# jepsen-io/maelstrom

Hardware: AMD Instinct MI355X
Metric: simulated_msgs_per_sec (histories/sec passing checker in histories_per_sec) (higher is better)
Workload: dtype u32

## Files before the change

maelstrom_amd/csrc/checker.hip:

```cpp
#include <hip/hip_runtime.h>

#include <cstring>
#include <vector>

#include "engine_internal.h"

#define NONE 0xFFFFu
#define NONE32 0xFFFFFFFFu
#define NOLAT 0xFFFFFFFFu

struct CParams {
  const msim_op *rows;
  const u32 *payload;
  const msim_inst_meta *meta;
  msim_check_result *out;
  u32 *recs;
  u32 max_rows, max_pay, max_values, C, workload, max_reads;
  u32 off_valid, off_tbl;
  float rcp_C;
};

#ifdef MSIM_HIPEMU
struct __attribute__((packed, aligned(4))) ck_u32x4 { u32 x, y, z, w; };
#else
// ... 339 lines not shown
      while (lo < hi) {
        const u32 mid = lo + (hi - lo) / 2;
        u32 c = 0;
        for (u32 e = lane; e < v_cur; e += 64) { const u32 l = lat[e]; c += (l != NOLAT && l <= mid) ? 1u : 0u; }
        if (c_wave_sum(c) > want) hi = mid; else lo = mid + 1;
      }
      q[qi] = lo;
    }
  }

  if (lane == 0) {
    msim_check_result o;
    o.attempt_count = v_cur; o.stable_count = n_stable; o.lost_count = n_lost; o.never_read_count = n_never;
    o.stale_count = n_stale; o.duplicated_count = 0; o.error_count = errors;
    for (int i = 0; i < 5; i++) o.stable_latency_ms[i] = q[i];
#ifdef CK_PROF
    o.stable_latency_ms[0] = (u32)(ck_t1 - ck_t0); o.stable_latency_ms[1] = (u32)(ck_t2 - ck_t1); o.stable_latency_ms[2] = (u32)(__builtin_readcyclecounter() - ck_t2); o.stable_latency_ms[3] = ck_rounds; o.stable_latency_ms[4] = n_ri;
#endif
    o.op_count = op_count; o.ok_count = n_ok; o.fail_count = n_fail; o.info_count = n_info;
    if (meta.flags) o.valid = 0;
    else if (!setfull) o.valid = errors == 0 ? 1 : 0;
    else o.valid = n_lost ? 0u : (n_stable == 0 ? 2u : 1u);
    p.out[inst] = o;
  }
}

static size_t check_lds_layout(CParams &cp) {
  size_t lds = (size_t)cp.max_values * 3 * 2 < (size_t)cp.max_values * 4 ? (size_t)cp.max_values * 4 : (size_t)cp.max_values * 3 * 2;
  lds = (lds + 3) & ~(size_t)3;
  cp.off_valid = (u32)lds;
  lds += ((size_t)(cp.max_reads + 31) / 32 + 2) * 4;
  cp.off_tbl = (u32)lds;
  lds += (size_t)cp.C * 3 * 4;
  return lds;
}

static const char *check_limits(u32 max_rows, u32 max_values, u32 concurrency) {
  if (max_rows >= 0xFFFF || max_values > 2048 || concurrency > 128 || concurrency == 0) return "device checker: max_rows must be < 65535, max_values <= 2048, concurrency 1..128";
  return nullptr;
}

static hipError_t check_dispatch(CParams &cp, u32 n, hipStream_t st) {
  cp.max_reads = cp.max_rows / 2 + 1;
  cp.rcp_C = 1.0f / (float)cp.C;
  const size_t lds = check_lds_layout(cp);
  if (lds > 64 * 1024) {
    const hipError_t e = hipFuncSetAttribute(reinterpret_cast<const void *>(&check_kernel), hipFuncAttributeMaxDynamicSharedMemorySize, (int)lds);
    if (e != hipSuccess) return e;
  }
  hipLaunchKernelGGL(check_kernel, dim3(n), dim3(64), lds, st, cp);
  return hipGetLastError();
}

int msim_check_launch(msim_ctx *ctx) {
  MSIM_HIP_TRY(ctx, hipSetDevice(ctx->device));
  const msim_config &c = ctx->cfg;
  CParams cp;
  std::memset(&cp, 0, sizeof cp);
  cp.rows = ctx->d_rows; cp.payload = ctx->d_payload; cp.meta = ctx->d_meta; cp.out = ctx->d_check;
  cp.max_rows = c.max_rows; cp.max_pay = c.max_payload_words; cp.max_values = c.max_values; cp.C = c.concurrency; cp.workload = c.workload;
  if (const char *why = check_limits(c.max_rows, c.max_values, c.concurrency)) { ctx->err = why; return MSIM_E_UNSUPPORTED; }
  const size_t rec_bytes = (size_t)ctx->n_inst * (c.max_rows / 2 + 1) * 3 * sizeof(u32);
  if (ctx->cap_check_scratch < rec_bytes) {
    if (ctx->d_check_scratch) (void)msim_dev_free(ctx->d_check_scratch);
    ctx->d_check_scratch = nullptr; ctx->cap_check_scratch = 0;
    MSIM_HIP_TRY(ctx, msim_dev_malloc(&ctx->d_check_scratch, rec_bytes));
    ctx->cap_check_scratch = rec_bytes;
  }
  cp.recs = static_cast<u32 *>(ctx->d_check_scratch);
  MSIM_HIP_TRY(ctx, hipEventRecord(ctx->ev2, ctx->stream));
  MSIM_HIP_TRY(ctx, check_dispatch(cp, ctx->n_inst, ctx->stream));
  MSIM_HIP_TRY(ctx, hipEventRecord(ctx->ev3, ctx->stream));
  MSIM_HIP_TRY(ctx, hipEventSynchronize(ctx->ev3));
  MSIM_HIP_TRY(ctx, hipEventElapsedTime(&ctx->check_ms, ctx->ev2, ctx->ev3));
  ctx->checked = true; ctx->check_fetched = false;
  return MSIM_OK;
}

extern "C" int msim_check_set_full_batch(int device, uint32_t workload, uint32_t concurrency, const msim_op *rows, const uint32_t *n_rows, uint32_t max_rows,
                                         const uint32_t *payload, uint32_t max_payload_words, uint32_t max_values, uint32_t n_histories, msim_check_result *out) {
  if (!rows || !n_rows || !out || n_histories == 0 || max_rows == 0 || (!payload && max_payload_words)) return MSIM_E_INVALID;
  if (workload != MSIM_WL_ECHO && workload != MSIM_WL_BROADCAST && workload != MSIM_WL_G_SET) return MSIM_E_INVALID;
  if (check_limits(max_rows, max_values, concurrency)) return MSIM_E_UNSUPPORTED;
  if (hipSetDevice(device) != hipSuccess) return MSIM_E_HIP;
  std::vector<msim_inst_meta> hm(n_histories);
  for (u32 i = 0; i < n_histories; i++) { std::memset(&hm[i], 0, sizeof hm[i]); if (n_rows[i] > max_rows) return MSIM_E_RANGE; hm[i].n_rows = n_rows[i]; }
  CParams cp;
  std::memset(&cp, 0, sizeof cp);
  cp.max_rows = max_rows; cp.max_pay = max_payload_words; cp.max_values = max_values; cp.C = concurrency; cp.workload = workload;
  msim_op *d_rows = nullptr; u32 *d_pay = nullptr; msim_inst_meta *d_meta = nullptr; msim_check_result *d_out = nullptr; u32 *d_rec = nullptr;
  const size_t pay_bytes = (size_t)n_histories * (max_payload_words ? max_payload_words : 1) * sizeof(u32);
  int rc = MSIM_E_HIP;
  do {
    if (msim_dev_malloc(&d_rows, (size_t)n_histories * max_rows * sizeof(msim_op)) != hipSuccess) break;
    if (msim_dev_malloc(&d_pay, pay_bytes) != hipSuccess) break;
    if (msim_dev_malloc(&d_meta, (size_t)n_histories * sizeof(msim_inst_meta)) != hipSuccess) break;
    if (msim_dev_malloc(&d_out, (size_t)n_histories * sizeof(msim_check_result)) != hipSuccess) break;
    if (msim_dev_malloc(&d_rec, (size_t)n_histories * (max_rows / 2 + 1) * 3 * sizeof(u32)) != hipSuccess) break;
    if (hipMemcpy(d_rows, rows, (size_t)n_histories * max_rows * sizeof(msim_op), hipMemcpyHostToDevice) != hipSuccess) break;
    if (max_payload_words && hipMemcpy(d_pay, payload, pay_bytes, hipMemcpyHostToDevice) != hipSuccess) break;
    if (hipMemcpy(d_meta, hm.data(), (size_t)n_histories * sizeof(msim_inst_meta), hipMemcpyHostToDevice) != hipSuccess) break;
    cp.rows = d_rows; cp.payload = d_pay; cp.meta = d_meta; cp.out = d_out; cp.recs = d_rec;
    if (check_dispatch(cp, n_histories, nullptr) != hipSuccess) break;
    if (hipDeviceSynchronize() != hipSuccess) break;
    if (hipMemcpy(out, d_out, (size_t)n_histories * sizeof(msim_check_result), hipMemcpyDeviceToHost) != hipSuccess) break;
    rc = MSIM_OK;
  } while (false);
  for (void *q : {(void *)d_rows, (void *)d_pay, (void *)d_meta, (void *)d_out, (void *)d_rec}) if (q) (void)msim_dev_free(q);
  return rc;
}

__global__ void __launch_bounds__(64) availability_kernel(const msim_op *rows, const msim_inst_meta *meta, u32 max_rows, uint2 *out) {
  const u32 lane = threadIdx.x, inst = blockIdx.x;
  const u32 n = meta[inst].n_rows;
  const uint4 *r = reinterpret_cast<const uint4 *>(rows + (size_t)inst * max_rows);
  u32 ok = 0, inv = 0;
  for (u32 i = lane; i < n; i += 64) { const u32 t = r[i].z & 3u; ok += t == MSIM_T_OK; inv += t == MSIM_T_INVOKE; }
  ok = c_wave_sum(ok); inv = c_wave_sum(inv);
  if (lane == 0) out[inst] = make_uint2(ok, inv);
}

static void availability_verdict(uint32_t ok, uint32_t inv, uint32_t mode, double a, msim_availability *o) {
  o->ok_count = ok; o->invoke_count = inv;
  o->ok_fraction = inv == 0 ? 1.0f : (float)((double)ok / (double)inv);
  o->valid = mode == MSIM_AVAIL_NIL ? 1u : mode == MSIM_AVAIL_TOTAL ? (o->ok_fraction == 1.0f ? 1u : 0u) : (a <= (double)o->ok_fraction ? 1u : 0u);
}

extern "C" int msim_check_availability_rows(const msim_op *rows, uint32_t n_rows, uint32_t mode, double availability, msim_availability *out) {
  if ((!rows && n_rows) || !out || mode > MSIM_AVAIL_FRACTION || (mode == MSIM_AVAIL_FRACTION && !(availability >= 0.0 && availability <= 1.0))) return MSIM_E_INVALID;
// ... 27 lines not shown
```

maelstrom_amd/csrc/engine.hip:

```cpp
#include <hip/hip_runtime.h>
#include <cstdlib>

#include <cstdio>
#include <cstring>
#include <new>
#include <vector>


#include "sim_kernels.h"

__device__ u32 wave_min_ref(u32 v) { for (int o = 32; o; o >>= 1) v = min(v, (u32)__shfl_xor((int)v, o)); return v; }
__device__ u32 wave_incl_scan_ref(u32 v) {
  const u32 lane = threadIdx.x & 63;
  for (int o = 1; o < 64; o <<= 1) { u32 t = (u32)__shfl_up((int)v, o); if (lane >= (u32)o) v += t; }
  return v;
}
__global__ void wave_selftest_kernel(const u32 *in, u32 *out) {
  const u32 lane = threadIdx.x;
  const u32 v = in[blockIdx.x * 64 + lane];
  u32 bad = 0;
  bad |= wave_min(v) != wave_min_ref(v);
  bad |= wave_incl_scan(v & 0xFFFF) != wave_incl_scan_ref(v & 0xFFFF);
  bad |= wave_sum(v & 0xFF) != rdlane(wave_incl_scan_ref(v & 0xFF), 63);
  bad |= (lane < 32) && scan32(v & 0xFFFF) != wave_incl_scan_ref(v & 0xFFFF);
// ... 37 lines not shown
  if (c->d_gpay) (void)msim_dev_free(c->d_gpay);
  if (c->d_goff) (void)msim_dev_free(c->d_goff);
  c->d_grows = c->d_gpay = nullptr; c->d_goff = nullptr; c->cap_grows = c->cap_gpay = c->cap_goff = 0;
  c->d_compact = nullptr; c->d_off = nullptr;
  c->cap_compact = c->cap_off = c->cap_h_rows = c->cap_h_payload = c->cap_h_journal = c->cap_h_meta = 0;
  delete[] c->h_row_off; delete[] c->h_pay_off; delete[] c->h_ev_off;
  c->d_journal = nullptr; c->h_journal = nullptr; c->h_ev_off = nullptr;
  c->d_rows = nullptr; c->d_payload = nullptr; c->d_stats = nullptr; c->d_meta = nullptr; c->d_scratch = nullptr; c->d_check = nullptr;
  c->h_rows = nullptr; c->h_payload = nullptr; c->h_stats = nullptr; c->h_meta = nullptr; c->h_check = nullptr;
  c->h_row_off = nullptr; c->h_pay_off = nullptr;
  c->cap_inst = 0;
}

extern "C" int msim_create(const msim_config *cfg, int device, msim_ctx **out, char *err, size_t errlen) {
  if (!cfg || !out) { set_err(err, errlen, "null argument"); return MSIM_E_INVALID; }
  *out = nullptr;
  msim_config c = *cfg;
  int rc = msim_config_finalize(&c, err, errlen);
  if (rc != MSIM_OK) return rc;
  const bool dt_many = (c.node_program == MSIM_NODE_TXN_DATOMIC || c.node_program == MSIM_NODE_TXN_MULTI_KEY) && c.concurrency > c.n_nodes;
  if ((c.node_program == MSIM_NODE_TXN_MULTI_KEY || c.node_program == MSIM_NODE_TXN_DATOMIC) && !dt_many && (c.concurrency != c.n_nodes || c.n_nodes > 30)) {
    set_err(err, errlen, "multi_key_txn / datomic: one worker per node and at most 30 nodes (two service lanes), or k x node-count workers with nodes + workers + 2 <= 64");
    return MSIM_E_UNSUPPORTED;
  }
  if (dt_many && c.n_nodes + c.concurrency + 2 > 64) { set_err(err, errlen, "multi_key_txn / datomic with several workers per node: nodes + workers + 2 services <= 64"); return MSIM_E_UNSUPPORTED; }
  const bool txn_many = (c.node_program == MSIM_NODE_TXN_SINGLE_KEY || c.node_program == MSIM_NODE_KAFKA) && c.concurrency > c.n_nodes;
  if (c.node_program == MSIM_NODE_BCAST_BATCH && (c.n_nodes > 32 || c.n_nodes + (c.concurrency > c.n_nodes ? c.concurrency : c.n_nodes) > 64)) {
    set_err(err, errlen, "broadcast-batch: one cluster per wavefront only: n_nodes <= 32 and n_nodes + max(concurrency, n_nodes) <= 64");
    return MSIM_E_UNSUPPORTED;
  }
  const uint32_t slots = (c.concurrency > c.n_nodes ? c.concurrency : c.n_nodes) + (dt_many ? 2 : txn_many ? 1 : 0);
  const bool wide_prog = c.node_program == MSIM_NODE_G_SET || c.node_program == MSIM_NODE_BCAST_FF || c.node_program == MSIM_NODE_BCAST_FF_ECHOBACK ||
                         c.node_program == MSIM_NODE_BCAST_ACK_RETRY || c.node_program == MSIM_NODE_BCAST_RPC_ALL || c.node_program == MSIM_NODE_PN_COUNTER;
  const bool wide = c.n_nodes > 32 && c.n_nodes <= 127 && wide_prog && c.concurrency == c.n_nodes;
  const uint32_t svc_lanes = c.node_program == MSIM_NODE_LIN_KV_PROXY || c.node_program == MSIM_NODE_TSO_IDS ? 1 : 0;
  if (!wide && (c.n_nodes > 32 || c.n_nodes + slots + svc_lanes > 64)) {
    set_err(err, errlen, "this build maps one cluster to one wavefront: n_nodes <= 32 and n_nodes + max(concurrency, n_nodes) <= 64 "
                         "(g-set, the counters and the broadcast programs with concurrency == n_nodes: up to 127 nodes)");
    return MSIM_E_UNSUPPORTED;
  }
  int ndev = 0;
  if (hipGetDeviceCount(&ndev) != hipSuccess || ndev <= 0) {
    set_err(err, errlen, "no HIP device visible: libmaelsim has no CPU path"); return MSIM_E_NO_DEVICE; }
  if (device < 0 || device >= ndev) { set_err(err, errlen, "device index out of range"); return MSIM_E_INVALID; }
  msim_ctx *ctx = new (std::nothrow) msim_ctx();
  if (!ctx) return MSIM_E_NOMEM;
  ctx->cfg = c; ctx->device = device;
  hipError_t e = hipSetDevice(device);
  if (e == hipSuccess) e = hipStreamCreateWithFlags(&ctx->stream, hipStreamNonBlocking);
  if (e == hipSuccess) e = hipEventCreate(&ctx->ev0);
  if (e == hipSuccess) e = hipEventCreate(&ctx->ev1);
  if (e == hipSuccess) e = hipEventCreate(&ctx->ev2);
  if (e == hipSuccess) e = hipEventCreate(&ctx->ev3);
  if (e != hipSuccess) { set_err(err, errlen, hipGetErrorString(e)); delete ctx; return MSIM_E_HIP; }
  *out = ctx;
  return MSIM_OK;
}

static uint32_t mk_tcap(const msim_config &c) {
  const double ops = (double)c.rate_mhz * (double)c.time_limit_ms / 1e6 * 1.125 + 64.0;
  uint32_t t = 64; while (t < 4.0 * ops * c.max_txn_length / c.n_nodes + 64.0) t <<= 1;
  return t;
}
static uint32_t mk_ccap(const msim_config &c) { return 4 * mk_tcap(c); }

static uint32_t raft_log_cap(const msim_config &c) {
  const double expected = (double)c.rate_mhz * (double)c.time_limit_ms / 1e6;
  return (uint32_t)(expected + expected / 8.0) + 64 + 8;
}
static uint64_t proto_scratch_words(const msim_config &c) {
  uint64_t w = 4;
  if (c.node_program == MSIM_NODE_RAFT) w = (uint64_t)c.n_nodes * raft_log_cap(c) * 2 + (uint64_t)c.n_nodes * R_ARENA_WORDS;
  if (c.node_program == MSIM_NODE_BCAST_ACK_RETRY) w = (uint64_t)c.n_nodes * c.max_values * 3;
  if (c.node_program == MSIM_NODE_BCAST_BATCH) w = (uint64_t)c.n_nodes * (c.max_values / 2) + (uint64_t)c.n_nodes * c.n_nodes * 4;
  if (c.node_program == MSIM_NODE_TXN_SINGLE_KEY) w = (uint64_t)c.max_values * (c.max_writes_per_key + 1);
  if (c.node_program == MSIM_NODE_TXN_MULTI_KEY)
    w = (uint64_t)c.max_values * (c.max_writes_per_key + 4 + 2 * (c.max_writes_per_key + 1)) + (uint64_t)c.n_nodes * mk_ccap(c) + (uint64_t)c.n_nodes * mk_tcap(c) / 4 + 4 +
        (uint64_t)c.n_nodes * ((c.concurrency > c.n_nodes ? MKG_SLOTS : MK_SLOTS) - MK_SL) * mk_slot_words(8);
  if (c.node_program == MSIM_NODE_TXN_DATOMIC) w = dt_scratch_words(c);
  if (c.node_program == MSIM_NODE_KAFKA) w = (uint64_t)KF_KEYS * (2 * (c.max_writes_per_key + 1) + 1);
  if (c.node_program == MSIM_NODE_TXN_RW_HAT) {
    const uint64_t G = c.max_rows / 2;
    w = (uint64_t)c.n_nodes * c.max_values + 2 * G + ((uint64_t)c.n_nodes * G + 3) / 4 + c.replication_words;
  }
  if (c.node_program == MSIM_NODE_G_SET || c.node_program == MSIM_NODE_PN_COUNTER) {
    const uint64_t total_ms = (uint64_t)c.time_limit_ms + c.quiesce_ms + 2ull * c.client_timeout_ms;
    const uint64_t ticks = total_ms / 5000 + 3;
    w = ticks * c.n_nodes * (c.max_values / 32);
    if (c.n_nodes > 32) w = ((w + ticks * (c.max_values / 32) + 3) & ~3ull) + (c.node_program == MSIM_NODE_G_SET ? wide_sparse_words(ticks, c.max_values / 32) : 0) + (((uint64_t)c.n_nodes * (c.max_values / 32) + 3) & ~3ull);
  }
  const bool bcast_ff = c.node_program == MSIM_NODE_BCAST_FF || c.node_program == MSIM_NODE_BCAST_FF_ECHOBACK;
  const bool bcast_rpc = c.node_program == MSIM_NODE_BCAST_ACK_RETRY || c.node_program == MSIM_NODE_BCAST_RPC_ALL;
  if (bcast_ff && c.n_nodes > 32) w = 4 + (((uint64_t)c.n_nodes * (c.max_values / 32) + 3) & ~3ull);
  if (bcast_rpc && c.n_nodes > 32) w = (uint64_t)c.n_nodes * c.max_values * 6 + (((uint64_t)c.n_nodes * (c.max_values / 32) + 3) & ~3ull);
  return (w + 3) & ~3ull;
}
static uint64_t scratch_words(const msim_config &c) {
  const uint64_t queues = c.n_nodes + (c.node_program == MSIM_NODE_KAFKA || c.node_program == MSIM_NODE_TXN_SINGLE_KEY || c.node_program == MSIM_NODE_LIN_KV_PROXY || c.node_program == MSIM_NODE_TSO_IDS ? 1 : c.node_program == MSIM_NODE_TXN_MULTI_KEY || c.node_program == MSIM_NODE_TXN_DATOMIC ? 2 : 0);
  uint64_t w = proto_scratch_words(c) + queues * c.spill_capacity * 4;
  if (c.node_program == MSIM_NODE_LIN_KV_PROXY || c.node_program == MSIM_NODE_TSO_IDS) w += (uint64_t)(c.concurrency > c.n_nodes ? c.concurrency : c.n_nodes) * (R_CLIENT_CAP - PX_CL) * 4;
  if (msim_raft4_eligible(c)) w += msim_raft4_extra_scratch_words(c);
  if (msim_svc4_eligible(c)) w += msim_svc4_extra_scratch_words(c);
  if (msim_txng4_eligible(c)) w += msim_txng4_extra_scratch_words(c);
  if (msim_dtg4_eligible(c)) w += msim_dtg4_extra_scratch_words(c);
  if (msim_txn8_eligible(c)) w += msim_txn8_extra_scratch_words(c);
  if (msim_mk8_eligible(c)) w += msim_mk8_extra_scratch_words(c);
  if (msim_dt8_eligible(c)) w += msim_dt8_extra_scratch_words(c);
  if (msim_hat8_eligible(c)) w += msim_hat8_extra_scratch_words(c);
  if (msim_kafka8_eligible(c)) w += msim_kafka8_extra_scratch_words(c);
  if (msim_uid8_eligible(c)) w += msim_uid8_extra_scratch_words(c);
  if (msim_crdt8_eligible(c)) w += msim_crdt8_extra_scratch_words(c);
  if (msim_bcast8_eligible(c)) w += msim_bcast8_extra_scratch_words(c);
  if (msim_duo_eligible(c)) w = ((w + 31) & ~31ull) + msim_duo_extra_scratch_words(c);
  return w;
}

static int ensure_buffers(msim_ctx *ctx, uint32_t n) {
  if (n <= ctx->cap_inst) return MSIM_OK;
  free_buffers(ctx);
  const msim_config &c = ctx->cfg;
  ctx->scratch_words_per_inst = scratch_words(c);
  MSIM_HIP_TRY(ctx, msim_dev_malloc(&ctx->d_rows, (size_t)n * c.max_rows * sizeof(msim_op)));
  MSIM_HIP_TRY(ctx, msim_dev_malloc(&ctx->d_payload, (size_t)n * c.max_payload_words * 4));
  MSIM_HIP_TRY(ctx, msim_dev_malloc(&ctx->d_stats, (size_t)n * sizeof(msim_net_stats)));
  MSIM_HIP_TRY(ctx, msim_dev_malloc(&ctx->d_meta, (size_t)n * sizeof(msim_inst_meta)));
  MSIM_HIP_TRY(ctx, msim_dev_malloc(&ctx->d_scratch, (size_t)n * ctx->scratch_words_per_inst * 4));
  MSIM_HIP_TRY(ctx, msim_dev_malloc(&ctx->d_check, (size_t)n * sizeof(msim_check_result)));
  if (c.journal_capacity) MSIM_HIP_TRY(ctx, msim_dev_malloc(&ctx->d_journal, (size_t)n * c.journal_capacity * sizeof(msim_event)));
  ctx->cap_inst = n;
  return MSIM_OK;
}

static int run_impl(msim_ctx *ctx, uint64_t first, uint32_t n, hipStream_t st, bool blocking) {
  if (!ctx) return MSIM_E_INVALID;
  if (n == 0) { ctx->err = "n_instances must be > 0"; return MSIM_E_INVALID; }
  MSIM_HIP_TRY(ctx, hipSetDevice(ctx->device));
  if (ctx->fetch_pending) { MSIM_HIP_TRY(ctx, hipStreamSynchronize(ctx->stream)); ctx->fetch_pending = false; }
  int rc = ensure_buffers(ctx, n);
  if (rc != MSIM_OK) return rc;
  const msim_config &c = ctx->cfg;
  KParams kp;
  std::memset(&kp, 0, sizeof kp);
  kp.cfg = c; kp.first_instance = first;
  kp.rows = ctx->d_rows; kp.payload = ctx->d_payload; kp.stats = ctx->d_stats; kp.meta = ctx->d_meta;
  kp.scratch = ctx->d_scratch; kp.scratch_words = ctx->scratch_words_per_inst;
  kp.journal = reinterpret_cast<uint4 *>(ctx->d_journal);
  kp.N = c.n_nodes; kp.C = c.concurrency; kp.CS = c.concurrency > c.n_nodes ? c.concurrency : c.n_nodes;
  kp.W = c.max_values / 32;
  kp.cap_node = c.inbox_capacity; kp.spill_cap = c.spill_capacity; kp.spill_off = proto_scratch_words(c);
  const uint64_t period_us = 1000000000ull / (c.rate_mhz ? c.rate_mhz : 1);
  if (2 * period_us > 0xFFFFFFFFull || 2000ull * c.nemesis_interval_ms > 0xFFFFFFFFull) { ctx->err = "rate too low / nemesis interval too long for u32 microseconds"; return MSIM_E_INVALID; }
  kp.gen_period2_us = (u32)(2 * period_us);
  kp.nem_period2_us = (u32)(2000ull * c.nemesis_interval_ms);
  const bool is_raft = c.node_program == MSIM_NODE_RAFT;
  kp.raft_log_cap = is_raft ? raft_log_cap(c) : 0;
  kp.dev_flags = msim_dev_flags(ctx);
  const bool wide = c.n_nodes > 32;
  const bool wide_setl = wide_sets_in_lds(c, kp.dev_flags);
  const bool wide_crdt = wide && (c.node_program == MSIM_NODE_G_SET || c.node_program == MSIM_NODE_PN_COUNTER);
  size_t off = (wide_setl || wide_crdt) ? 0 : (wide ? WIDE_STAGE_ROWS : STAGE_ROWS) * 16;
  const bool is_txn = c.node_program == MSIM_NODE_TXN_SINGLE_KEY, is_px = c.node_program == MSIM_NODE_LIN_KV_PROXY || c.node_program == MSIM_NODE_TSO_IDS;
  const bool is_hat = c.node_program == MSIM_NODE_TXN_RW_HAT, is_mk = c.node_program == MSIM_NODE_TXN_MULTI_KEY, is_kf = c.node_program == MSIM_NODE_KAFKA, is_dt = c.node_program == MSIM_NODE_TXN_DATOMIC;
  kp.mk_tcap = is_mk ? mk_tcap(c) : is_dt ? dt_tcap(c) : 0; kp.mk_ccap = is_mk ? mk_ccap(c) : 0;
  kp.off_inbox = (u32)off;
  const bool dt_many = (is_dt || is_mk) && c.concurrency > c.n_nodes;
  const bool txn_many = (is_txn || is_kf) && c.concurrency > c.n_nodes;
  off += (is_mk || is_dt) ? ((size_t)(kp.N + 2) * kp.cap_node + (size_t)(dt_many ? kp.CS : kp.N) * T_CLIENT_CAP) * 16 : is_hat ? ((size_t)kp.N * kp.cap_node + (size_t)kp.CS * T_CLIENT_CAP) * 16    : is_px ? ((size_t)(kp.N + 1) * kp.cap_node + (size_t)kp.CS * PX_CL) * 16 : (is_txn || is_kf) ? ((size_t)(kp.N + 1) * kp.cap_node + (size_t)(txn_many ? kp.CS : kp.N) * T_CLIENT_CAP) * 16
                : ((size_t)kp.N * kp.cap_node + (size_t)kp.CS * (is_raft ? R_CLIENT_CAP : CLIENT_INBOX_CAP)) * 16 + wide_client_bytes(c);
  kp.off_seen = (u32)off;
  off += is_mk ? ((size_t)kp.N * MK_SL * mk_slot_words(mk_keys_for(c)) + (size_t)kp.N * mk_keys_for(c) * 3 + 36) * 4
       : is_dt ? ((size_t)kp.N * (dt_many ? DG_WORDS : DC_WORDS) + 36) * 4
       : is_hat ? 36 * 4
       : is_px ? (size_t)kp.N * PX_SLOTS * 8 + ((c.node_program == MSIM_NODE_LIN_KV_PROXY && c.proxy_service == MSIM_SVC_SEQ_KV) ? 34 : 2) * 256 + 64 * 4
       : is_txn ? (size_t)kp.N * (txn_many ? TG_SLOTS : TXN_SLOTS) * 16 + 36 * 4
       : is_kf ? ((size_t)kp.N * (txn_many ? KFG_SLOTS : KF_SLOTS) * KSW + (size_t)kp.N * KF_KEYS + (size_t)(txn_many ? kp.CS : kp.N) * KF_KEYS + 36 + 2 * KF_KEYS) * 4
       : is_raft ? (size_t)kp.N * 256 + (size_t)kp.N * kp.N * 3 * 4
       : wide ? (wide_setl ? (size_t)kp.N * kp.W * 4 : 0) + wide_pending_bytes(c)
                 : (size_t)kp.N * kp.W * 4;
  off = (off + 15) & ~(size_t)15;
  kp.off_misc = (u32)off; if (c.nemesis_mask) off += (wide ? 128 : 64) * 4;
  const size_t lds = off;
  if (lds > 160 * 1024) { ctx->err = "cluster state exceeds the 160 KiB LDS of a CU (lower inbox_capacity / max_values)"; return MSIM_E_INVALID; }

  static const int poison = []() { const char *p = std::getenv("MSIM_POISON"); return p ? (int)(std::strtoul(p, nullptr, 0) & 0xFFu) : -1; }();
  if (poison >= 0) {
    MSIM_HIP_TRY(ctx, hipMemsetAsync(ctx->d_rows, poison, (size_t)ctx->cap_inst * c.max_rows * sizeof(msim_op), st));
    MSIM_HIP_TRY(ctx, hipMemsetAsync(ctx->d_payload, poison, (size_t)ctx->cap_inst * c.max_payload_words * 4, st));
    MSIM_HIP_TRY(ctx, hipMemsetAsync(ctx->d_stats, poison, (size_t)ctx->cap_inst * sizeof(msim_net_stats), st));
    MSIM_HIP_TRY(ctx, hipMemsetAsync(ctx->d_meta, poison, (size_t)ctx->cap_inst * sizeof(msim_inst_meta), st));
    MSIM_HIP_TRY(ctx, hipMemsetAsync(ctx->d_scratch, poison, (size_t)ctx->cap_inst * ctx->scratch_words_per_inst * 4, st));
    MSIM_HIP_TRY(ctx, hipMemsetAsync(ctx->d_check, poison, (size_t)ctx->cap_inst * sizeof(msim_check_result), st));
    if (ctx->d_journal) MSIM_HIP_TRY(ctx, hipMemsetAsync(ctx->d_journal, poison, (size_t)ctx->cap_inst * c.journal_capacity * sizeof(msim_event), st));
    if (ctx->d_check_scratch) MSIM_HIP_TRY(ctx, hipMemsetAsync(ctx->d_check_scratch, poison, ctx->cap_check_scratch, st));
    if (ctx->d_perf_scratch) MSIM_HIP_TRY(ctx, hipMemsetAsync(ctx->d_perf_scratch, poison, ctx->cap_perf_scratch, st));
  }
  MSIM_HIP_TRY(ctx, hipEventRecord(ctx->ev0, st));
  hipError_t e;
  const char *kname = "?";
  auto took = [&](hipError_t r, const char *k) { if (r != MSIM_LAYOUT_DOES_NOT_FIT) kname = k; return r; };
  e = MSIM_LAYOUT_DOES_NOT_FIT;
  if (msim_duo_eligible(c) && !(kp.dev_flags & 0x200u) && !((kp.dev_flags & 0x8000u) && msim_bcast8_eligible(c))) {
    e = took(msim_launch_duo(kp, n, st), "duo");
    if (e == MSIM_LAYOUT_DOES_NOT_FIT && (kp.dev_flags & 0x400u)) { ctx->err = "MSIM_DEV_FLAGS bit 10: the two-clusters-per-wavefront layout was required but this cluster state does not fit it"; return MSIM_E_UNSUPPORTED; }
  }
  if (e == MSIM_LAYOUT_DOES_NOT_FIT && msim_bcast8_eligible(c) && !(kp.dev_flags & 0x200u)) e = took(msim_launch_bcast8(kp, n, st), "bcast8");
  if (msim_raft4_eligible(c) && !(kp.dev_flags & 0x200u)) e = took(msim_launch_raft4(kp, n, st), "raft4");
  if (msim_svc4_eligible(c) && !(kp.dev_flags & 0x200u)) e = took(msim_launch_svc4(kp, n, st), c.node_program == MSIM_NODE_TSO_IDS ? "svc4<TSO>" : "svc4");
  if (msim_txng4_eligible(c) && !(kp.dev_flags & 0x200u)) e = took(msim_launch_txng4(kp, n, st), "txng4");
  if (msim_dtg4_eligible(c) && !(kp.dev_flags & 0x200u)) e = took(msim_launch_dtg4(kp, n, st), "dtg4");
  if (msim_txn8_eligible(c) && !(kp.dev_flags & 0x200u)) e = took(msim_launch_txn8(kp, n, st), "txn8");
  if (msim_mk8_eligible(c) && !(kp.dev_flags & 0x200u)) e = took(msim_launch_mk8(kp, n, st), "mk8");
  if (msim_dt8_eligible(c) && !(kp.dev_flags & 0x200u)) e = took(msim_launch_dt8(kp, n, st), "dt8");
  if (msim_hat8_eligible(c) && !(kp.dev_flags & 0x200u)) e = took(msim_launch_hat8(kp, n, st), "hat8");
  if (msim_kafka8_eligible(c) && !(kp.dev_flags & 0x200u)) e = took(msim_launch_kafka8(kp, n, st), "kafka8");
  if (msim_uid8_eligible(c) && !(kp.dev_flags & 0x200u)) e = took(msim_launch_uid8(kp, n, st), "uid8");
  if (msim_crdt8_eligible(c) && !(kp.dev_flags & 0x200u)) e = took(msim_launch_crdt8(kp, n, st), "crdt8");
  if (e == MSIM_LAYOUT_DOES_NOT_FIT && (kp.dev_flags & 0x400u) && is_raft) { ctx->err = "MSIM_DEV_FLAGS bit 10: the four-clusters-per-wavefront Raft layout was required but does not apply"; return MSIM_E_UNSUPPORTED; }
  if (e == MSIM_LAYOUT_DOES_NOT_FIT) switch (c.node_program) {
    case MSIM_NODE_ECHO: case MSIM_NODE_FLAKE_IDS: e = took(msim_launch_general_a(kp, n, lds, st), "general_a"); break;
    case MSIM_NODE_G_SET: e = wide ? took(msim_launch_wide_gset(kp, n, lds, st), "wide_gset") : took(msim_launch_general_a(kp, n, lds, st), "general_a"); break;
    case MSIM_NODE_PN_COUNTER: e = wide ? took(msim_launch_wide_pn(kp, n, lds, st), "wide_pn") : took(msim_launch_general_a(kp, n, lds, st), "general_a"); break;
    case MSIM_NODE_BCAST_FF: case MSIM_NODE_BCAST_FF_ECHOBACK: e = wide ? took(msim_launch_wide_bcast(kp, n, lds, st), "wide_bcast") : took(msim_launch_general_b(kp, n, lds, st), "general_b"); break;
    case MSIM_NODE_BCAST_ACK_RETRY: case MSIM_NODE_BCAST_RPC_ALL: e = wide ? took(msim_launch_wide_ack(kp, n, lds, st), "wide_ack") : took(msim_launch_general_c(kp, n, lds, st), "general_c"); break;
    case MSIM_NODE_BCAST_BATCH: e = took(msim_launch_general_d(kp, n, lds, st), "general_d"); break;
    case MSIM_NODE_RAFT: e = took(msim_launch_raft1(kp, n, lds, st), "raft1"); break;
    case MSIM_NODE_LIN_KV_PROXY: case MSIM_NODE_TSO_IDS: e = took(msim_launch_svc1(kp, n, lds, st), "svc1"); break;
    case MSIM_NODE_TXN_SINGLE_KEY: e = txn_many ? took(msim_launch_txng(kp, n, lds, st), "txng") : took(msim_launch_txn1(kp, n, lds, st), "txn1"); break;
    case MSIM_NODE_TXN_MULTI_KEY: e = dt_many ? took(msim_launch_mkg(kp, n, lds, st), "mkg") : took(msim_launch_mk1(kp, n, lds, st), "mk1"); break;
    case MSIM_NODE_TXN_DATOMIC: e = dt_many ? took(msim_launch_dtg(kp, n, lds, st), "dtg") : took(msim_launch_dt1(kp, n, lds, st), "dt1"); break;
    case MSIM_NODE_KAFKA: e = txn_many ? took(msim_launch_kafkag(kp, n, lds, st), "kafkag") : took(msim_launch_kafka1(kp, n, lds, st), "kafka1"); break;
    case MSIM_NODE_TXN_RW_HAT: e = c.concurrency > c.n_nodes ? took(msim_launch_hatg(kp, n, lds, st), "hatg") : took(msim_launch_hat1(kp, n, lds, st), "hat1"); break;
    default: ctx->err = "node program not built into this engine"; return MSIM_E_UNSUPPORTED;
  }
  if (kp.dev_flags & 0x1000u) std::fprintf(stderr, "[layout] %s %u\n", kname, n);
  if (e != hipSuccess) { ctx->err = std::string("kernel launch: ") + hipGetErrorString(e); return MSIM_E_HIP; }
  ctx->n_inst = n; ctx->first_instance = first;
  ctx->fetched = false; ctx->fetch_pending = false; ctx->checked = false; ctx->check_fetched = false; ctx->ran = true;
  MSIM_HIP_TRY(ctx, hipEventRecord(ctx->ev1, st));
  ctx->sim_ms_stale = true;
  if (blocking) {
    MSIM_HIP_TRY(ctx, hipEventSynchronize(ctx->ev1));
    MSIM_HIP_TRY(ctx, hipEventElapsedTime(&ctx->sim_ms, ctx->ev0, ctx->ev1));
    ctx->sim_ms_stale = false;
  }
  return MSIM_OK;
}

extern "C" int msim_run(msim_ctx *ctx, uint64_t first_instance, uint32_t n_instances) {
  if (!ctx) return MSIM_E_INVALID;
  return run_impl(ctx, first_instance, n_instances, ctx->stream, true);
}

extern "C" int msim_run_async(msim_ctx *ctx, uint64_t first_instance, uint32_t n_instances, void *hip_stream) {
  if (!ctx) return MSIM_E_INVALID;
  return run_impl(ctx, first_instance, n_instances, hip_stream ? (hipStream_t)hip_stream : ctx->stream, false);
}

extern "C" int msim_check(msim_ctx *ctx) {
  if (!ctx) return MSIM_E_INVALID;
  if (!ctx->ran) { ctx->err = "msim_check before msim_run"; return MSIM_E_RANGE; }
  if (ctx->cfg.workload == MSIM_WL_LIN_KV) {
    return (msim_dev_flags(ctx) & 0x800u) ?
           msim_check_lin_kv_host(ctx) : msim_check_lin_kv_device(ctx);
  }
  if (ctx->cfg.workload == MSIM_WL_TXN_LIST_APPEND) {
    return (msim_dev_flags(ctx) & 0x800u) ?
           msim_check_txn_host(ctx) : msim_check_txn_device(ctx);
  }
  if (ctx->cfg.workload == MSIM_WL_TXN_RW_REGISTER) {
    return (msim_dev_flags(ctx) & 0x800u) ?
           msim_check_txn_host(ctx) : msim_check_rw_device(ctx);
  }
  if (ctx->cfg.workload == MSIM_WL_KAFKA) {
    return (msim_dev_flags(ctx) & 0x800u) ?
           msim_check_kafka_host(ctx) : msim_check_kafka_device(ctx);
  }
  if (ctx->cfg.workload == MSIM_WL_PN_COUNTER || ctx->cfg.workload == MSIM_WL_G_COUNTER) {
    return (msim_dev_flags(ctx) & 0x800u) ?
           msim_check_pn_host(ctx) : msim_check_pn_device(ctx);
  }
  if (ctx->cfg.workload == MSIM_WL_UNIQUE_IDS) {
    return (msim_dev_flags(ctx) & 0x800u) ?
           msim_check_unique_host(ctx) : msim_check_unique_device(ctx);
  }
  return msim_check_launch(ctx);
}

__global__ void __launch_bounds__(256) compact_kernel(const uint4 *__restrict__ src, uint4 *__restrict__ dst, const uint64_t *__restrict__ off,
                                                      uint64_t stride_units) {
  const u32 i = blockIdx.x;
  const uint64_t o = off[i], cnt = off[i + 1] - o;
  const uint4 *s = src + (size_t)i * stride_units;
  for (uint64_t k = (uint64_t)blockIdx.y * 256 + threadIdx.x; k < cnt; k += (uint64_t)gridDim.y * 256) dst[o + k] = s[k];
}
__global__ void __launch_bounds__(256) compact_words_kernel(const u32 *__restrict__ src, u32 *__restrict__ dst, const uint64_t *__restrict__ off,
                                                            uint64_t stride_words) {
  const u32 i = blockIdx.x;
  const uint64_t o = off[i], cnt = off[i + 1] - o;
  const u32 *s = src + (size_t)i * stride_words;
  for (uint64_t k = (uint64_t)blockIdx.y * 256 + threadIdx.x; k < cnt; k += (uint64_t)gridDim.y * 256) dst[o + k] = s[k];
}

template <typename T>
static int grow_pinned(msim_ctx *ctx, T **buf, size_t *cap, size_t bytes) {
  if (*buf && *cap >= bytes) return MSIM_OK;
  if (*buf) { (void)hipHostFree(*buf); *buf = nullptr; *cap = 0; }
  const size_t want = bytes + bytes / 8 + 4096;
  MSIM_HIP_TRY(ctx, hipHostMalloc(reinterpret_cast<void **>(buf), want));
  *cap = want;
  return MSIM_OK;
}

static int fetch_compacted(msim_ctx *ctx, const void *d_src, uint64_t stride_units, bool units16, const uint64_t *h_off, void *h_dst, int pair, int phase) {
  const uint32_t n = ctx->n_inst;
  const uint64_t total = h_off[n];
  if (!total) return MSIM_OK;
  void **d_compact = pair ? &ctx->d_compact2 : &ctx->d_compact; size_t *cap_compact = pair ? &ctx->cap_compact2 : &ctx->cap_compact;
  uint64_t **d_off = pair ? &ctx->d_off2 : &ctx->d_off; size_t *cap_off = pair ? &ctx->cap_off2 : &ctx->cap_off;
  const size_t unit = units16 ? 16 : 4, bytes = (size_t)total * unit;
  if (phase == 1) { MSIM_HIP_TRY(ctx, hipMemcpyAsync(h_dst, *d_compact, bytes, hipMemcpyDeviceToHost, ctx->stream)); return MSIM_OK; }
  if (*cap_compact < bytes) {
    if (*d_compact) (void)msim_dev_free(*d_compact);
    *d_compact = nullptr; *cap_compact = 0;
    MSIM_HIP_TRY(ctx, msim_dev_malloc(d_compact, bytes + bytes / 8));
    *cap_compact = bytes + bytes / 8;
  }
  if (*cap_off < (size_t)(n + 1) * 8) {
    if (*d_off) (void)msim_dev_free(*d_off);
    *d_off = nullptr; *cap_off = 0;
    MSIM_HIP_TRY(ctx, msim_dev_malloc(reinterpret_cast<void **>(d_off), (size_t)(n + 1) * 8));
    *cap_off = (size_t)(n + 1) * 8;
  }
  MSIM_HIP_TRY(ctx, hipMemcpyAsync(*d_off, h_off, (size_t)(n + 1) * 8, hipMemcpyHostToDevice, ctx->stream));
  const uint64_t avg = total / n + 1;
  const unsigned gy = (unsigned)((avg + 1023) / 1024 < 1 ? 1 : ((avg + 1023) / 1024 > 64 ? 64 : (avg + 1023) / 1024));
  if (units16) hipLaunchKernelGGL(compact_kernel, dim3(n, gy), dim3(256), 0, ctx->stream, static_cast<const uint4 *>(d_src), static_cast<uint4 *>(*d_compact), *d_off, stride_units);
  else hipLaunchKernelGGL(compact_words_kernel, dim3(n, gy), dim3(256), 0, ctx->stream, static_cast<const u32 *>(d_src), static_cast<u32 *>(*d_compact), *d_off, stride_units);
// ... 144 lines not shown
  if (!ctx) return MSIM_E_INVALID;
  if (!ctx->checked) { ctx->err = "msim_check_results before msim_check"; return MSIM_E_RANGE; }
  if (!ctx->check_fetched) {
    MSIM_HIP_TRY(ctx, hipSetDevice(ctx->device));
    if (ctx->h_check) { (void)hipHostFree(ctx->h_check); ctx->h_check = nullptr; }
    MSIM_HIP_TRY(ctx, hipHostMalloc(&ctx->h_check, (size_t)ctx->n_inst * sizeof(msim_check_result)));
    MSIM_HIP_TRY(ctx, hipMemcpy(ctx->h_check, ctx->d_check, (size_t)ctx->n_inst * sizeof(msim_check_result), hipMemcpyDeviceToHost));
    ctx->check_fetched = true;
  }
  if (results) *results = ctx->h_check;
  if (n) *n = ctx->n_inst;
  return MSIM_OK;
}

extern "C" int msim_device_buffers_get(msim_ctx *ctx, msim_device_buffers *out) {
  if (!ctx || !out) return MSIM_E_INVALID;
  if (!ctx->ran) { ctx->err = "no run yet"; return MSIM_E_RANGE; }
  const msim_config &c = ctx->cfg;
  out->rows = ctx->d_rows; out->payload = ctx->d_payload; out->stats = ctx->d_stats; out->meta = ctx->d_meta;
  out->check = ctx->d_check; out->check_bytes = (uint64_t)ctx->n_inst * sizeof(msim_check_result);
  out->journal = ctx->d_journal; out->journal_bytes = (uint64_t)ctx->n_inst * c.journal_capacity * sizeof(msim_event);
  out->rows_bytes = (uint64_t)ctx->n_inst * c.max_rows * sizeof(msim_op);
  out->payload_bytes = (uint64_t)ctx->n_inst * c.max_payload_words * 4;
  out->stats_bytes = (uint64_t)ctx->n_inst * sizeof(msim_net_stats);
  out->meta_bytes = (uint64_t)ctx->n_inst * sizeof(msim_inst_meta);
  out->n_instances = ctx->n_inst; out->max_rows = c.max_rows; out->max_payload_words = c.max_payload_words; out->journal_capacity = c.journal_capacity;
  return MSIM_OK;
}

extern "C" int msim_last_kernel_ms(msim_ctx *ctx, float *sim_ms, float *check_ms) {
  if (!ctx) return MSIM_E_INVALID;
  if (ctx->sim_ms_stale) {
    MSIM_HIP_TRY(ctx, hipSetDevice(ctx->device));
    MSIM_HIP_TRY(ctx, hipEventSynchronize(ctx->ev1));
    MSIM_HIP_TRY(ctx, hipEventElapsedTime(&ctx->sim_ms, ctx->ev0, ctx->ev1));
    ctx->sim_ms_stale = false;
  }
  if (sim_ms) *sim_ms = ctx->sim_ms;
  if (check_ms) *check_ms = ctx->check_ms;
  return MSIM_OK;
}

extern "C" int msim_get_config(const msim_ctx *ctx, msim_config *out) {
  if (!ctx || !out) return MSIM_E_INVALID;
  *out = ctx->cfg;
  return MSIM_OK;
}

extern "C" const char *msim_last_error(const msim_ctx *ctx) { return ctx ? ctx->err.c_str() : "null ctx"; }

extern "C" void msim_destroy(msim_ctx *ctx) {
  if (!ctx) return;
  (void)hipSetDevice(ctx->device);
  free_buffers(ctx);
  msim_gather_free(ctx);
  if (ctx->ev0) (void)hipEventDestroy(ctx->ev0);
  if (ctx->ev1) (void)hipEventDestroy(ctx->ev1);
  if (ctx->ev2) (void)hipEventDestroy(ctx->ev2);
  if (ctx->ev3) (void)hipEventDestroy(ctx->ev3);
  if (ctx->stream) (void)hipStreamDestroy(ctx->stream);
  delete ctx;
}

extern "C" int msim_selftest_wave(int device) {
  if (hipSetDevice(device) != hipSuccess) return MSIM_E_NO_DEVICE;
  const int blocks = 64, n = blocks * 64;
  u32 *h = new u32[n], *d_in = nullptr, *d_out = nullptr;
  u64 x = 12345;
  for (int i = 0; i < n; i++) { x = mix64(x + i); h[i] = (u32)x; if (i % 7 == 0) h[i] = 0xFFFFFFFFu; }
  int bad = 0;
  if (msim_dev_malloc(&d_in, n * 4) != hipSuccess || msim_dev_malloc(&d_out, n * 4) != hipSuccess) { delete[] h; return MSIM_E_HIP; }
  (void)hipMemcpy(d_in, h, n * 4, hipMemcpyHostToDevice);
  hipLaunchKernelGGL(wave_selftest_kernel, dim3(blocks), dim3(64), 0, 0, d_in, d_out);
  if (hipMemcpy(h, d_out, n * 4, hipMemcpyDeviceToHost) != hipSuccess) bad = MSIM_E_HIP;
  else for (int i = 0; i < n; i++) bad += h[i] != 0;
  (void)msim_dev_free(d_in); (void)msim_dev_free(d_out);
  delete[] h;
  return bad;
}
```

maelstrom_amd/csrc/engine_internal.h:

```cpp
#ifndef MSIM_ENGINE_INTERNAL_H
#define MSIM_ENGINE_INTERNAL_H

#include <hip/hip_runtime.h>
#include <string>

#include "../../include/maelsim.h"
#include "engine_limits.h"

typedef uint32_t u32;
typedef uint64_t u64;

struct msim_ctx {
  msim_config cfg{};
  int device = 0;
  hipStream_t stream = nullptr;
  hipEvent_t ev0 = nullptr, ev1 = nullptr, ev2 = nullptr, ev3 = nullptr;
  hipEvent_t ev_g0 = nullptr, ev_g1 = nullptr;
  uint32_t n_inst = 0, cap_inst = 0;
  uint64_t first_instance = 0;
  msim_op *d_rows = nullptr;
  uint32_t *d_payload = nullptr;
  msim_net_stats *d_stats = nullptr;
  msim_inst_meta *d_meta = nullptr;
  uint32_t *d_scratch = nullptr;
  uint64_t scratch_words_per_inst = 0;
  msim_check_result *d_check = nullptr;
  msim_event *d_journal = nullptr;
  msim_op *h_rows = nullptr;
  uint32_t *h_payload = nullptr;
  msim_net_stats *h_stats = nullptr;
  msim_inst_meta *h_meta = nullptr;
  msim_check_result *h_check = nullptr;
  msim_event *h_journal = nullptr;
  uint64_t *h_row_off = nullptr, *h_pay_off = nullptr, *h_ev_off = nullptr;
  void *d_check_scratch = nullptr; size_t cap_check_scratch = 0;
  void *d_perf_scratch = nullptr; size_t cap_perf_scratch = 0;
  void *d_compact = nullptr; uint64_t *d_off = nullptr;
  void *d_compact2 = nullptr; uint64_t *d_off2 = nullptr; size_t cap_compact2 = 0, cap_off2 = 0;
  bool fetch_pending = false;
  size_t cap_compact = 0, cap_off = 0, cap_h_rows = 0, cap_h_payload = 0, cap_h_journal = 0, cap_h_meta = 0;
  void *comm = nullptr; int comm_rank = 0, comm_world = 1;
  void *d_grows = nullptr, *d_gpay = nullptr; uint64_t *d_goff = nullptr; size_t cap_grows = 0, cap_gpay = 0, cap_goff = 0;
  uint64_t g_row_units = 0, g_pay_words = 0;
  void *d_all[4] = {nullptr, nullptr, nullptr, nullptr}; size_t cap_all[4] = {0, 0, 0, 0};
  uint64_t *d_sizes = nullptr;
  bool fetched = false, checked = false, check_fetched = false, ran = false;
  float sim_ms = 0.f, check_ms = 0.f;
  bool sim_ms_stale = false;
  uint32_t dev_flags = 0;
  uint32_t txn_big = 0;
  uint32_t lin_host_rechecks = 0;
  bool check_classify = false;
  std::string err;
};

#include <cstdio>
#include <cstdlib>
#include <thread>
static inline unsigned msim_host_threads() {
  if (const char *e = std::getenv("MSIM_HOST_THREADS")) { const int v = std::atoi(e); if (v > 0) return (unsigned)v; }
  unsigned nt = std::thread::hardware_concurrency();
  if (nt == 0) nt = 1;
  if (std::FILE *f = std::fopen("/sys/fs/cgroup/cpu.max", "r")) {
    long long q = 0, per = 0;
    if (std::fscanf(f, "%lld %lld", &q, &per) == 2 && q > 0 && per > 0) { const unsigned lim = (unsigned)((q + per - 1) / per); if (lim >= 1 && lim < nt) nt = lim; }
    std::fclose(f);
  }
  if (const char *e = std::getenv("LOCAL_WORLD_SIZE")) { const int v = std::atoi(e); if (v > 1) nt = nt / (unsigned)v ? nt / (unsigned)v : 1; }
  return nt;
}

static inline uint32_t msim_dev_flags(const msim_ctx *ctx) {
  static const uint32_t env = []() { const char *e = std::getenv("MSIM_DEV_FLAGS"); return e ? (uint32_t)std::strtoul(e, nullptr, 0) : 0u; }();
  return env | (ctx ? ctx->dev_flags : 0u);
}

int msim_compact_on_device(msim_ctx *ctx, uint64_t *row_units, uint64_t *pay_words);
void msim_gather_free(msim_ctx *ctx);
int msim_check_launch(msim_ctx *ctx);
int msim_check_lin_kv_host(msim_ctx *ctx, msim_lin_key_result *keys = nullptr, uint32_t max_keys = 0, uint32_t *n_keys = nullptr);
int msim_check_lin_kv_device(msim_ctx *ctx, msim_lin_key_result *keys = nullptr, uint32_t max_keys = 0, uint32_t *n_keys = nullptr);
int msim_check_txn_host(msim_ctx *ctx);
int msim_check_txn_device(msim_ctx *ctx);
int msim_check_rw_device(msim_ctx *ctx);
int msim_check_kafka_host(msim_ctx *ctx);
int msim_check_kafka_device(msim_ctx *ctx);
int msim_check_unique_device(msim_ctx *ctx);
int msim_check_pn_device(msim_ctx *ctx);
int msim_check_pn_host(msim_ctx *ctx);
int msim_check_unique_host(msim_ctx *ctx);

hipError_t msim_dev_malloc_impl(void **out, size_t bytes);
hipError_t msim_dev_free(void *ptr);
template <typename T> static inline hipError_t msim_dev_malloc(T **out, size_t bytes) { return msim_dev_malloc_impl(reinterpret_cast<void **>(out), bytes); }

#define MSIM_HIP_TRY(ctx, call)                                                        \
  do {                                                                                 \
    hipError_t e_ = (call);                                                            \
    if (e_ != hipSuccess) {                                                            \
      (ctx)->err = std::string(#call) + ": " + hipGetErrorString(e_);                 \
      return MSIM_E_HIP;                                                               \
    }                                                                                  \
  } while (0)

#endif
```

Before: 453.8 billion.

## Enqueue checker kernel right after simulation when a prior check was requested

Splits the checker launch into reserve/enqueue/wait. Once a check has been requested on the context's own stream, later runs of the echo/broadcast/g-set workloads enqueue the checker immediately after the simulation kernel, and the later check call only waits on the event. This removes the host round-trip and launch gap between simulation and check. It also records an event on the null stream and makes the run wait on it. The catch is that a check is speculatively queued even when the caller never asks for one.

```diff
diff --git a/maelstrom_amd/csrc/checker.hip b/maelstrom_amd/csrc/checker.hip
--- a/maelstrom_amd/csrc/checker.hip
+++ b/maelstrom_amd/csrc/checker.hip
@@ -415,7 +415,18 @@
   return hipGetLastError();
 }
 
-int msim_check_launch(msim_ctx *ctx) {
+int msim_check_reserve(msim_ctx *ctx, uint32_t n) {
+  const size_t rec_bytes = (size_t)n * (ctx->cfg.max_rows / 2 + 1) * 3 * sizeof(u32);
+  if (ctx->cap_check_scratch < rec_bytes) {
+    if (ctx->d_check_scratch) (void)msim_dev_free(ctx->d_check_scratch);
+    ctx->d_check_scratch = nullptr; ctx->cap_check_scratch = 0;
+    MSIM_HIP_TRY(ctx, msim_dev_malloc(&ctx->d_check_scratch, rec_bytes));
+    ctx->cap_check_scratch = rec_bytes;
+  }
+  return MSIM_OK;
+}
+
+int msim_check_enqueue(msim_ctx *ctx, hipStream_t stream) {
   MSIM_HIP_TRY(ctx, hipSetDevice(ctx->device));
   const msim_config &c = ctx->cfg;
   CParams cp;
@@ -423,21 +434,26 @@
   cp.rows = ctx->d_rows; cp.payload = ctx->d_payload; cp.meta = ctx->d_meta; cp.out = ctx->d_check;
   cp.max_rows = c.max_rows; cp.max_pay = c.max_payload_words; cp.max_values = c.max_values; cp.C = c.concurrency; cp.workload = c.workload;
   if (const char *why = check_limits(c.max_rows, c.max_values, c.concurrency)) { ctx->err = why; return MSIM_E_UNSUPPORTED; }
-  const size_t rec_bytes = (size_t)ctx->n_inst * (c.max_rows / 2 + 1) * 3 * sizeof(u32);
-  if (ctx->cap_check_scratch < rec_bytes) {
-    if (ctx->d_check_scratch) (void)msim_dev_free(ctx->d_check_scratch);
-    ctx->d_check_scratch = nullptr; ctx->cap_check_scratch = 0;
-    MSIM_HIP_TRY(ctx, msim_dev_malloc(&ctx->d_check_scratch, rec_bytes));
-    ctx->cap_check_scratch = rec_bytes;
-  }
+  const int rc = msim_check_reserve(ctx, ctx->n_inst);
+  if (rc != MSIM_OK) return rc;
   cp.recs = static_cast<u32 *>(ctx->d_check_scratch);
-  MSIM_HIP_TRY(ctx, hipEventRecord(ctx->ev2, ctx->stream));
-  MSIM_HIP_TRY(ctx, check_dispatch(cp, ctx->n_inst, ctx->stream));
-  MSIM_HIP_TRY(ctx, hipEventRecord(ctx->ev3, ctx->stream));
+  MSIM_HIP_TRY(ctx, hipEventRecord(ctx->ev2, stream));
+  MSIM_HIP_TRY(ctx, check_dispatch(cp, ctx->n_inst, stream));
+  MSIM_HIP_TRY(ctx, hipEventRecord(ctx->ev3, stream));
+  return MSIM_OK;
+}
+
+int msim_check_wait(msim_ctx *ctx) {
+  MSIM_HIP_TRY(ctx, hipSetDevice(ctx->device));
   MSIM_HIP_TRY(ctx, hipEventSynchronize(ctx->ev3));
   MSIM_HIP_TRY(ctx, hipEventElapsedTime(&ctx->check_ms, ctx->ev2, ctx->ev3));
   ctx->checked = true; ctx->check_fetched = false;
   return MSIM_OK;
+}
+
+int msim_check_launch(msim_ctx *ctx) {
+  const int rc = msim_check_enqueue(ctx, ctx->stream);
+  return rc != MSIM_OK ? rc : msim_check_wait(ctx);
 }
 
 extern "C" int msim_check_set_full_batch(int device, uint32_t workload, uint32_t concurrency, const msim_op *rows, const uint32_t *n_rows, uint32_t max_rows,
diff --git a/maelstrom_amd/csrc/engine.hip b/maelstrom_amd/csrc/engine.hip
--- a/maelstrom_amd/csrc/engine.hip
+++ b/maelstrom_amd/csrc/engine.hip
@@ -113,6 +113,7 @@
   if (e == hipSuccess) e = hipEventCreate(&ctx->ev1);
   if (e == hipSuccess) e = hipEventCreate(&ctx->ev2);
   if (e == hipSuccess) e = hipEventCreate(&ctx->ev3);
+  if (e == hipSuccess) e = hipEventCreateWithFlags(&ctx->ev_null, hipEventDisableTiming);
   if (e != hipSuccess) { set_err(err, errlen, hipGetErrorString(e)); delete ctx; return MSIM_E_HIP; }
   *out = ctx;
   return MSIM_OK;
@@ -192,14 +193,25 @@
   return MSIM_OK;
 }
 
+static bool check_launch_route(const msim_config &c) {
+  return c.workload == MSIM_WL_ECHO || c.workload == MSIM_WL_BROADCAST || c.workload == MSIM_WL_G_SET;
+}
+
 static int run_impl(msim_ctx *ctx, uint64_t first, uint32_t n, hipStream_t st, bool blocking) {
   if (!ctx) return MSIM_E_INVALID;
   if (n == 0) { ctx->err = "n_instances must be > 0"; return MSIM_E_INVALID; }
   MSIM_HIP_TRY(ctx, hipSetDevice(ctx->device));
   if (ctx->fetch_pending) { MSIM_HIP_TRY(ctx, hipStreamSynchronize(ctx->stream)); ctx->fetch_pending = false; }
+  const bool own_stream = st == ctx->stream;
+  if (ctx->check_queued) {
+    ctx->check_queued = false; ctx->check_armed = false;
+    if (!own_stream) MSIM_HIP_TRY(ctx, hipStreamSynchronize(ctx->stream));
+  }
   int rc = ensure_buffers(ctx, n);
   if (rc != MSIM_OK) return rc;
   const msim_config &c = ctx->cfg;
+  const bool queue_check = ctx->check_armed && own_stream && check_launch_route(c) && !(msim_dev_flags(ctx) & 0x40000u) &&
+                           msim_check_reserve(ctx, n) == MSIM_OK;
   KParams kp;
   std::memset(&kp, 0, sizeof kp);
   kp.cfg = c; kp.first_instance = first;
@@ -243,6 +255,10 @@
   const size_t lds = off;
   if (lds > 160 * 1024) { ctx->err = "cluster state exceeds the 160 KiB LDS of a CU (lower inbox_capacity / max_values)"; return MSIM_E_INVALID; }
 
+  if (own_stream) {
+    MSIM_HIP_TRY(ctx, hipEventRecord(ctx->ev_null, nullptr));
+    MSIM_HIP_TRY(ctx, hipStreamWaitEvent(st, ctx->ev_null, 0));
+  }
   static const int poison = []() { const char *p = std::getenv("MSIM_POISON"); return p ? (int)(std::strtoul(p, nullptr, 0) & 0xFFu) : -1; }();
   if (poison >= 0) {
     MSIM_HIP_TRY(ctx, hipMemsetAsync(ctx->d_rows, poison, (size_t)ctx->cap_inst * c.max_rows * sizeof(msim_op), st));
@@ -297,8 +313,13 @@
   if (e != hipSuccess) { ctx->err = std::string("kernel launch: ") + hipGetErrorString(e); return MSIM_E_HIP; }
   ctx->n_inst = n; ctx->first_instance = first;
   ctx->fetched = false; ctx->fetch_pending = false; ctx->checked = false; ctx->check_fetched = false; ctx->ran = true;
+  ctx->ran_own_stream = own_stream;
   MSIM_HIP_TRY(ctx, hipEventRecord(ctx->ev1, st));
   ctx->sim_ms_stale = true;
+  if (queue_check) {
+    ctx->check_queued = msim_check_enqueue(ctx, st) == MSIM_OK;
+    if (ctx->check_queued && (kp.dev_flags & 0x1000u)) std::fprintf(stderr, "[check] queued %u\n", n);
+  }
   if (blocking) {
     MSIM_HIP_TRY(ctx, hipEventSynchronize(ctx->ev1));
     MSIM_HIP_TRY(ctx, hipEventElapsedTime(&ctx->sim_ms, ctx->ev0, ctx->ev1));
@@ -344,6 +365,14 @@
     return (msim_dev_flags(ctx) & 0x800u) ?
            msim_check_unique_host(ctx) : msim_check_unique_device(ctx);
   }
+  const uint32_t flags = msim_dev_flags(ctx);
+  if (ctx->check_queued) {
+    ctx->check_queued = false;
+    if (flags & 0x1000u) std::fprintf(stderr, "[check] taken %u\n", ctx->n_inst);
+    return msim_check_wait(ctx);
+  }
+  if (ctx->ran_own_stream && !(flags & 0x40000u)) ctx->check_armed = true;
+  if (flags & 0x1000u) std::fprintf(stderr, "[check] launched %u\n", ctx->n_inst);
   return msim_check_launch(ctx);
 }
 
@@ -594,12 +623,14 @@
 extern "C" void msim_destroy(msim_ctx *ctx) {
   if (!ctx) return;
   (void)hipSetDevice(ctx->device);
+  if (ctx->check_queued && ctx->stream) (void)hipStreamSynchronize(ctx->stream);
   free_buffers(ctx);
   msim_gather_free(ctx);
   if (ctx->ev0) (void)hipEventDestroy(ctx->ev0);
   if (ctx->ev1) (void)hipEventDestroy(ctx->ev1);
   if (ctx->ev2) (void)hipEventDestroy(ctx->ev2);
   if (ctx->ev3) (void)hipEventDestroy(ctx->ev3);
+  if (ctx->ev_null) (void)hipEventDestroy(ctx->ev_null);
   if (ctx->stream) (void)hipStreamDestroy(ctx->stream);
   delete ctx;
 }
diff --git a/maelstrom_amd/csrc/engine_internal.h b/maelstrom_amd/csrc/engine_internal.h
--- a/maelstrom_amd/csrc/engine_internal.h
+++ b/maelstrom_amd/csrc/engine_internal.h
@@ -16,6 +16,7 @@
   hipStream_t stream = nullptr;
   hipEvent_t ev0 = nullptr, ev1 = nullptr, ev2 = nullptr, ev3 = nullptr;
   hipEvent_t ev_g0 = nullptr, ev_g1 = nullptr;
+  hipEvent_t ev_null = nullptr;
   uint32_t n_inst = 0, cap_inst = 0;
   uint64_t first_instance = 0;
   msim_op *d_rows = nullptr;
@@ -45,6 +46,7 @@
   void *d_all[4] = {nullptr, nullptr, nullptr, nullptr}; size_t cap_all[4] = {0, 0, 0, 0};
   uint64_t *d_sizes = nullptr;
   bool fetched = false, checked = false, check_fetched = false, ran = false;
+  bool ran_own_stream = false, check_armed = false, check_queued = false;
   float sim_ms = 0.f, check_ms = 0.f;
   bool sim_ms_stale = false;
   uint32_t dev_flags = 0;
@@ -77,6 +79,9 @@
 
 int msim_compact_on_device(msim_ctx *ctx, uint64_t *row_units, uint64_t *pay_words);
 void msim_gather_free(msim_ctx *ctx);
+int msim_check_reserve(msim_ctx *ctx, uint32_t n);
+int msim_check_enqueue(msim_ctx *ctx, hipStream_t stream);
+int msim_check_wait(msim_ctx *ctx);
 int msim_check_launch(msim_ctx *ctx);
 int msim_check_lin_kv_host(msim_ctx *ctx, msim_lin_key_result *keys = nullptr, uint32_t max_keys = 0, uint32_t *n_keys = nullptr);
 int msim_check_lin_kv_device(msim_ctx *ctx, msim_lin_key_result *keys = nullptr, uint32_t max_keys = 0, uint32_t *n_keys = nullptr);
```

Result: faster. 486.2 billion (median of 6 runs) (+7.2%).
